# 31415Hacker/RayTracer-public

Measured on AMD Instinct MI355X. Metric: Msamples/sec @1920x1080 Stanford-Dragon-class, 4 spp, 8 bounces, higher is better.
Workload: dtype f32; 1 GPU; C2: dragon-class procedural closed mesh (871414 tris, seed 20260109; dragon.glb absent), native LBVH2->BVH4, 1920x1080, 4 spp, 8 bounces, camera (0,0,2.5) identity quat FOV 70, a new frame index (sample set) every step; triangles=871414, bvh4_nodes=1263056, width=1920, height=1080, spp=4, max_bounces=8, seed=1, frames_per_launch=32

## Files before the change

include/mi355pt.h:

```cpp
#ifndef MI355PT_H
#define MI355PT_H

#include <stdint.h>

#ifdef __cplusplus
extern "C" {
#endif

#if defined(__GNUC__)
#define PT_API __attribute__((visibility("default")))
#else
#define PT_API
#endif

typedef struct PtContext PtContext;

typedef enum PtStatus {
    PT_OK = 0,
    PT_ERR_INVALID_ARG = 1,
    PT_ERR_NO_DEVICE = 2,
    PT_ERR_HIP = 3,
    PT_ERR_NO_SCENE = 4,
    PT_ERR_BAD_BVH = 5,
    PT_ERR_IO = 6,
// ... 183 lines not shown
PT_API int  pt_group_update_triangles(PtGroup* group, const float* tris, uint32_t num_tris);
PT_API int  pt_group_build_bvh(PtGroup* group);
PT_API int  pt_group_build_bvh_accel(PtGroup* group, uint32_t accel);
PT_API int  pt_group_set_bvh2(PtGroup* group, const uint32_t* bvh2, uint64_t words);
PT_API int  pt_group_set_bvh4(PtGroup* group, const uint32_t* bvh4, uint64_t words);
PT_API int  pt_group_set_batch(PtGroup* group, uint32_t frames_per_launch);
PT_API int  pt_group_render(PtGroup* group, const PtRenderParams* params);
PT_API int  pt_group_flush(PtGroup* group);
PT_API int  pt_group_synchronize(PtGroup* group);
PT_API int  pt_group_read_radiance(PtGroup* group, float* dst, uint64_t dst_floats);
PT_API int  pt_group_read_rgba8(PtGroup* group, uint8_t* dst, uint64_t dst_bytes);
PT_API int  pt_group_read_tonemapped(PtGroup* group, int from_rgba8, uint8_t* dst, uint64_t dst_bytes);

PT_API int pt_debug_set_tune(PtContext* ctx, const char* name, uint32_t value);
PT_API int pt_debug_launch_plan(uint32_t num_cus, uint32_t frames, uint32_t tile_count, uint32_t launches_in_flight, uint32_t traced_batches, uint32_t batch_size, uint32_t out[12]);
PT_API int pt_debug_counters(PtContext* ctx, unsigned long long* dst24);
PT_API int pt_debug_wave_times(PtContext* ctx, unsigned long long* dst, uint32_t max_waves, uint32_t* n_waves);
PT_API int pt_debug_traced_tiles(PtContext* ctx, const PtRenderParams* params, uint32_t* bitmask_out, uint32_t words, uint32_t* rect_tiles, uint32_t* traced_tiles);

#ifdef __cplusplus
}
#endif
#endif
```

raytracer-public_amd/__init__.py:

```python
import ctypes as C
import math
import os
import sys

import numpy as np

_HERE = os.path.dirname(os.path.abspath(__file__))
LIB_PATH = os.path.join(_HERE, "libmi355pt.so")

PT_MODE_REFERENCE_PACKET, PT_MODE_REFERENCE, PT_MODE_PATH = 0, 1, 2
PT_FLAG_STATS = 1
PT_FLAG_SIMPLE_KERNEL = 2
PT_FLAG_BRUTE_FORCE = 4
PT_FLAG_COMPACT = 8
SCENE_DRAGON_CLASS, SCENE_SPONZA_CLASS = 0, 1
PT_ACCEL_REFERENCE, PT_ACCEL_AREA_COLLAPSE, PT_ACCEL_PLOC = 0, 1, 2
PT_TRACE_ANY_HIT, PT_TRACE_STATS, PT_TRACE_SIMPLE_KERNEL = 1, 2, 4
PT_CLOSEST_STATS, PT_CLOSEST_SIMPLE_KERNEL, PT_CLOSEST_BRUTE_FORCE = 1, 2, 4
PT_OCCLUSION_STATS, PT_OCCLUSION_SIMPLE_KERNEL = 1, 2
PRIM_NONE = 0xFFFFFFFF


class PtError(RuntimeError):
    def __init__(self, code, message):
# ... 61 lines not shown
    "pt_compute_bvh2_sizing", "pt_compute_bvh4_sizing", "pt_morton_sort", "pt_collapse_lbvh2_to_bvh4",
    "pt_collapse_bvh2_to_bvh4_accel", "pt_build_bvh2_ploc", "pt_bvh2_to_bvh4_wide", "pt_file_write_u32", "pt_file_read_u32", "pt_scene_procedural",
    "pt_set_triangles", "pt_build_bvh", "pt_build_bvh_accel", "pt_build_lbvh2", "pt_read_bvh2", "pt_set_bvh4", "pt_set_bvh2",
    "pt_read_bvh4", "pt_set_spheres", "pt_scene_info", "pt_render", "pt_last_render_ms", "pt_set_batch", "pt_flush", "pt_timing_begin", "pt_timing_collect", "pt_timing_collect_spans", "pt_set_compact_buffer", "pt_set_output_buffer", "pt_get_stats", "pt_read_radiance",
    "pt_read_rgba8", "pt_read_tonemapped", "pt_tile_layout", "pt_tile_ids", "pt_compact_radiance", "pt_deinterleave", "pt_deinterleave_batch", "pt_buffer_busy",
    "pt_accum_info", "pt_read_accum", "pt_set_accum",
    "pt_trace_rays", "pt_trace_rays_host", "pt_camera_rays",
    "pt_closest_points", "pt_closest_points_host", "pt_closest_points_bvh4",
    "pt_occlusion", "pt_occlusion_host", "pt_occlusion_rays", "pt_occlusion_rays_host", "pt_hit_surfels", "pt_hit_surfels_host",
    "pt_update_triangles", "pt_update_triangles_device", "pt_bvh_cost", "pt_refit_bvh4", "pt_refit_bvh2", "pt_bvh4_cost", "pt_group_update_triangles",
    "pt_traced_tile_rect", "pt_packed_layout", "pt_packed_tile_ids", "pt_pack_shares", "pt_unpack_batch",
    "pt_group_create", "pt_group_destroy", "pt_group_last_error", "pt_group_size", "pt_group_context", "pt_group_set_triangles", "pt_group_build_bvh",
    "pt_group_build_bvh_accel",
    "pt_group_set_bvh2", "pt_group_set_bvh4", "pt_group_set_batch", "pt_group_render", "pt_group_flush", "pt_group_synchronize", "pt_group_read_radiance",
    "pt_group_read_rgba8", "pt_group_read_tonemapped",
    "pt_debug_set_tune", "pt_debug_counters", "pt_debug_wave_times", "pt_debug_launch_plan", "pt_debug_traced_tiles",
]


def _load():
    os.environ.setdefault("GPU_MAX_HW_QUEUES", "12")
    if not os.path.exists(LIB_PATH):
        raise ImportError(
            "libmi355pt.so is not built (%s). Run `python -c 'import __graft_entry__ as g; g.build()'` "
            "or `make -C raytracer-public_amd/csrc`. There is no CPU fallback." % LIB_PATH)
    lib = C.CDLL(LIB_PATH)
    lib.pt_last_error.restype = C.c_char_p
    lib.pt_last_error.argtypes = [C.c_void_p]
    lib.pt_version.restype = C.c_char_p
    lib.pt_destroy.restype = None
    lib.pt_destroy.argtypes = [C.c_void_p]
# ... 840 lines not shown
```

raytracer-public_amd/csrc/pt_api.cpp:

```cpp
#include "mi355pt.h"
#include "pt_host.h"
#include "pt_kernels.h"

#include <hip/hip_runtime.h>

#include <algorithm>
#include <cstdio>
#include <cstdlib>
#include <cstring>
#include <string>
#include <vector>

namespace {

thread_local std::string g_global_error;

template <typename T>
struct DevBuf {
    T* ptr = nullptr; size_t cap = 0;
    hipError_t ensure(size_t n) {
        if (n <= cap && ptr) return hipSuccess;
        if (ptr) { (void)hipFree(ptr); ptr = nullptr; cap = 0; }
        if (n == 0) n = 1;
        hipError_t e = hipMalloc((void**)&ptr, n * sizeof(T));
        if (e == hipSuccess) cap = n;
        return e;
    }
    void release() { if (ptr) (void)hipFree(ptr); ptr = nullptr; cap = 0; }
};

}

struct PtTune {
    static constexpr uint32_t kAuto = 0xFFFFFFFFu;
    uint32_t grid_div = kAuto, rows = kAuto, chunk = kAuto, xcd = kAuto, shade = kAuto, fill = kAuto,
             slots = kAuto, cull = kAuto, stats_batch = kAuto, quad = kAuto, fork = kAuto, bounded = kAuto, timeline = kAuto;
    uint32_t* find(const char* name) {
        static const struct { const char* n; uint32_t PtTune::* m; } tab[] = {
            {"GRIDDIV", &PtTune::grid_div}, {"ROWS", &PtTune::rows}, {"CHUNK", &PtTune::chunk}, {"XCD", &PtTune::xcd}, {"SHADE", &PtTune::shade},
            {"FILL", &PtTune::fill}, {"SLOTS", &PtTune::slots}, {"CULL", &PtTune::cull}, {"STATSBATCH", &PtTune::stats_batch}, {"QUAD", &PtTune::quad}, {"FORK", &PtTune::fork}, {"BOUNDED", &PtTune::bounded}, {"TIMELINE", &PtTune::timeline}};
        for (const auto& t : tab) if (std::strcmp(name, t.n) == 0) return &(this->*(t.m));
        return nullptr;
    }
    void from_environment() {
        static const char* names[] = {"GRIDDIV", "ROWS", "CHUNK", "XCD", "SHADE", "FILL", "SLOTS", "CULL", "STATSBATCH", "QUAD", "FORK", "BOUNDED", "TIMELINE"};
        for (const char* n : names) {
            const std::string key = std::string("PT_TUNE_") + n;
            const char* v = std::getenv(key.c_str());
            if (v && *v) *find(n) = uint32_t(std::strtoul(v, nullptr, 10));
        }
    }
    static uint32_t pick(uint32_t knob, uint32_t dflt) { return knob == kAuto ? dflt : knob; }
};

struct PtContext {
    int device = 0;
    PtTune tune;
    hipStream_t own_stream = nullptr;
    hipStream_t stream = nullptr;
    hipEvent_t ev_start = nullptr, ev_stop = nullptr;
// ... 63 lines not shown
    float4* ext_compact = nullptr; uint64_t ext_compact_floats = 0;
    float4* ext_out = nullptr; uint64_t ext_out_floats = 0;
    const float4* last_full = nullptr;
    bool last_stats = false;
    uint64_t stats_culled = 0;
    std::vector<hipEvent_t> ring;
    uint32_t ring_used = 0;
    struct InFlight { const char* lo; const char* hi; uint64_t seq; };
    std::vector<InFlight> inflight;
    uint64_t launch_seq = 0, delivered_seq = 0;
    hipEvent_t misc_fence = nullptr; uint64_t misc_fence_seq = 0;
};

namespace {

int fail(PtContext* ctx, int code, const std::string& msg) {
    if (ctx) ctx->err = msg; else g_global_error = msg;
    return code;
}
int fail_hip(PtContext* ctx, hipError_t e, const char* what) {
    return fail(ctx, PT_ERR_HIP, std::string(what) + ": " + hipGetErrorString(e));
}
#define PT_HIP(ctx, call) do { hipError_t e__ = (call); if (e__ != hipSuccess) return fail_hip((ctx), e__, #call); } while (0)

int bind(PtContext* ctx) {
    if (!ctx) return fail(nullptr, PT_ERR_INVALID_ARG, "null context");
    PT_HIP(ctx, hipSetDevice(ctx->device));
    return PT_OK;
}

// ... 60 lines not shown
    PT_HIP(ctx, hipMalloc((void**)&fresh, tri_bytes + (cap_nodes + 1u) * 64u));
    if (ctx->d_scene.ptr && ctx->scene_tris == num_tris && num_tris)
        PT_HIP(ctx, hipMemcpy(fresh, ctx->d_scene.ptr, uint64_t(num_tris) * 64u, hipMemcpyDeviceToDevice));
    if (ctx->d_scene.ptr) (void)hipFree(ctx->d_scene.ptr);
    PT_HIP(ctx, hipMemset((char*)fresh + uint64_t(num_tris) * 64u, 0, tri_bytes - uint64_t(num_tris) * 64u));
    ctx->d_scene.ptr = fresh; ctx->d_scene.cap = size_t((tri_bytes + (cap_nodes + 1u) * 64u) / 16u);
    ctx->node_off = tri_bytes; ctx->node_cap = cap_nodes; ctx->scene_tris = num_tris;
    return PT_OK;
}

int install_cut(PtContext* ctx) {
    ++ctx->tree_version; ctx->cut_count = 0;
    const uint32_t base16 = uint32_t(ctx->node_off / 16u), root = ctx->wide_meta.root_ref;
    if (root == pt::kInvalid || (root & pt::kLeafFlag) || ctx->num_wide == 0u || root < base16) return PT_OK;
    PT_HIP(ctx, ctx->d_cut.ensure(ptk::kCutMax + 1u));
    if (!ctx->h_word) PT_HIP(ctx, hipHostMalloc((void**)&ctx->h_word, 64, hipHostMallocDefault));
    PT_HIP(ctx, ptk::launch_tile_cut(ctx->wide(), ctx->num_wide, base16, (root - base16) / 4u, ctx->d_cut.ptr, ctx->stream));
    PT_HIP(ctx, hipMemcpyAsync(ctx->h_word, ctx->d_cut.ptr + ptk::kCutMax, 4, hipMemcpyDeviceToHost, ctx->stream));
    PT_HIP(ctx, hipStreamSynchronize(ctx->stream));
    ctx->cut_count = std::min(ctx->h_word[0], ptk::kCutMax);
    return PT_OK;
}

int upload_wide(PtContext* ctx, const uint32_t* bvh4, uint64_t words) {
    pt::WideBvh w; std::string err;
    if (int rc = sync_refit_meta(ctx)) return rc;
    const uint32_t tris_now = ctx->have_tris ? ctx->num_tris : 0u;
    if (!pt::build_wide_bvh(bvh4, words, tris_now, uint32_t(tri_region_bytes(tris_now) / 16u), w, err)) return fail(ctx, PT_ERR_BAD_BVH, err);
    PT_HIP(ctx, ctx->d_bvh4.ensure(words));
    PT_HIP(ctx, hipMemcpyAsync(ctx->d_bvh4.ptr, bvh4, words * 4, hipMemcpyHostToDevice, ctx->stream));
    if (int rc = ensure_scene(ctx, tris_now, w.nodes.size())) return rc;
// ... 50 lines not shown

struct PlanInput {
    uint32_t num_cus;
    uint32_t frames;
    uint32_t tile_count;
    bool     sharded;
    bool     stats;
    uint32_t launches_in_flight;
    uint32_t traced_batches;
    uint32_t batch_size;
};
struct LaunchPlan {
    uint32_t grid;
    uint32_t perm_rows, perm_cols, total_items, chunk_items, xcd_span;
    uint32_t shade_threshold, fill_threshold, quad_live, fork_shadow;
    int      slots, setup_slots;
    const char* error;
};

int slots_for(const PtTune& tune, uint32_t frames, uint32_t tile_count, bool sharded) {
    const uint32_t w8 = frames * 8u / (tile_count ? tile_count : 1u);
    const int n = int(PtTune::pick(tune.slots, w8 >= 256u ? 3u : (w8 >= 64u ? 4u : (w8 >= 16u ? PT_FRAME_SLOTS : (w8 >= 8u ? (sharded ? 4u : 6u) : (sharded ? 8u : PT_FRAME_SLOTS))))));
    return n < 1 ? 1 : (n > PtContext::kMaxSlots ? PtContext::kMaxSlots : n);
}

LaunchPlan plan_launch(const PtTune& tune, const PlanInput& in) {
    LaunchPlan P; std::memset(&P, 0, sizeof(P));
    const uint32_t nf = in.frames, count = in.tile_count ? in.tile_count : 1u;
    const int cus = in.num_cus > 0 ? int(in.num_cus) : 256;
    P.grid = ptk::megakernel_grid(cus);
// ... 6 lines not shown
    const uint32_t work8 = nf * 8u / count;
    P.perm_rows = PtTune::pick(tune.rows, work8 >= 24u ? nf : (work8 >= 8u ? 128u * nf : 64u * nf));
    if (P.perm_rows < 1u) P.perm_rows = 1u;
    if (P.perm_rows > 4096u) P.perm_rows = 4096u;
    P.perm_cols = (in.traced_batches + P.perm_rows - 1u) / P.perm_rows;
    if (uint64_t(P.perm_cols) * P.perm_rows * 64ull > 0xFFFFFFFFull) { P.error = "pt_render: batch too large (more than 2^32 items per launch)"; return P; }
    P.total_items = P.perm_cols * P.perm_rows * 64u;
    P.chunk_items = ((PtTune::pick(tune.chunk, 128u) + 63u) / 64u) * 64u;
    if (P.chunk_items < 64u) P.chunk_items = 64u;
    if (uint64_t(P.total_items) + uint64_t(grid_lanes / 64u + 1u) * P.chunk_items > 0xFFFFFFFFull) {
        P.error = "pt_render: launch too large for the 32-bit work-queue cursor (more than 2^32 - grid * chunk items; lower spp, the resolution or the batch)"; return P;
    }
    {
        const uint32_t per = (P.total_items + 7u) / 8u;
        P.xcd_span = PtTune::pick(tune.xcd, work8 >= 64u ? 1u : 0u) ? ((per + P.chunk_items - 1u) / P.chunk_items) * P.chunk_items : 0u;
    }
    P.shade_threshold = PtTune::pick(tune.shade, PT_SHADE_THRESHOLD); P.fill_threshold = PtTune::pick(tune.fill, PT_FILL_THRESHOLD);
    P.quad_live = std::min(16u, PtTune::pick(tune.quad, PT_QUAD_LIVE));
    P.fork_shadow = PtTune::pick(tune.fork, PT_FORK_SHADOW);
    P.slots = in.stats ? 1 : slots_for(tune, nf, count, in.sharded);
    P.setup_slots = in.stats ? 1 : std::max(P.slots, slots_for(tune, std::max(nf, in.batch_size), count, in.sharded));
    return P;
}

bool launch_rect(const PtContext* ctx, const ptk::FrameParams* frames, uint32_t nf, uint32_t width, uint32_t height, uint32_t num_tris, TileRect& rect) {
    rect = {0, 0, 0, 0};
    if (!(ctx->have_bvh && ctx->wide_meta.root_ref != pt::kInvalid && !ctx->wide_meta.root_degenerate && num_tris != 0u && ctx->tune.cull != 0u)) return false;
    for (uint32_t i = 0; i < nf; ++i) {
        TileRect r;
        if (!root_box_rect(ctx->wide_meta, frames[i], width, height, r)) return false;
// ... 48 lines not shown
        cv.cams = cams; cv.tree_version = ctx->tree_version; cv.width = width; cv.height = height;
        if (!now) return PT_OK;
    }
    if (!cv.computed) {
        if (int rc = sync_refit_meta(ctx)) return rc;
        const uint32_t tiles = ((width + pt::kTile - 1) / pt::kTile) * ((height + pt::kTile - 1) / pt::kTile), words = (tiles + 31u) / 32u;
        if (!ctx->cover_stream) {
            int lo = 0, hi = 0;
            (void)hipDeviceGetStreamPriorityRange(&lo, &hi);
            PT_HIP(ctx, hipStreamCreateWithPriority(&ctx->cover_stream, hipStreamNonBlocking, hi));
        }
        PT_HIP(ctx, ctx->d_cover.ensure(words + 1u));
        if (ctx->h_cover_cap < words + 1u) {
            if (ctx->h_cover) (void)hipHostFree(ctx->h_cover);
            ctx->h_cover = nullptr; ctx->h_cover_cap = 0;
            PT_HIP(ctx, hipHostMalloc((void**)&ctx->h_cover, (size_t(words) + 1u) * sizeof(uint32_t), hipHostMallocDefault));
            ctx->h_cover_cap = words + 1u;
        }
        cv.valid = false;
        PT_HIP(ctx, hipMemsetAsync(ctx->d_cover.ptr, 0, (size_t(words) + 1u) * sizeof(uint32_t), ctx->cover_stream));
        for (size_t first = 0; first < cams.size(); first += ptk::kCoverCams) {
            ptk::CoverCams group; std::memset(&group, 0, sizeof group);
            const uint32_t n = uint32_t(std::min<size_t>(ptk::kCoverCams, cams.size() - first));
            std::memcpy(group.c, cams.data() + first, n * sizeof(ptk::CoverCam));
            PT_HIP(ctx, ptk::launch_tile_cover(ctx->wide(), ctx->d_cut.ptr, ctx->cut_count, group, n, width, height, ctx->d_cover.ptr, words, ctx->cover_stream));
        }
        PT_HIP(ctx, hipMemcpyAsync(ctx->h_cover, ctx->d_cover.ptr, (size_t(words) + 1u) * sizeof(uint32_t), hipMemcpyDeviceToHost, ctx->cover_stream));
        PT_HIP(ctx, hipStreamSynchronize(ctx->cover_stream));
        cv.mask.assign(ctx->h_cover, ctx->h_cover + words);
        cv.usable = ctx->h_cover[words] == 0u;
        cv.id = ++ctx->cover_ids; if (cv.id == 0u) cv.id = ++ctx->cover_ids;
// ... 26 lines not shown
            PT_HIP(ctx, ptk::launch_prime(s.queue.ptr, s.side));
            s.primed_ptr = s.samples.ptr; s.primed_samples = cap_samples;
        }
    }
    return PT_OK;
}

int stage_traced_tiles(PtContext* ctx, PtContext::FrameSlot& sl, const uint32_t key[9], const std::vector<uint32_t>& traced, const uint32_t* cover, uint32_t words) {
    if (sl.cull_valid && std::memcmp(key, sl.cull_key, 9 * sizeof(uint32_t)) == 0) return PT_OK;
    if (!sl.trace_copied) PT_HIP(ctx, hipEventCreateWithFlags(&sl.trace_copied, hipEventDisableTiming));
    else PT_HIP(ctx, hipEventSynchronize(sl.trace_copied));
    const size_t need = traced.size() + words;
    if (sl.h_trace_cap < need) {
        if (sl.h_trace) (void)hipHostFree(sl.h_trace);
        sl.h_trace = nullptr; sl.h_trace_cap = 0;
        PT_HIP(ctx, hipHostMalloc((void**)&sl.h_trace, std::max<size_t>(need, 1024) * sizeof(uint32_t), hipHostMallocDefault));
        sl.h_trace_cap = std::max<size_t>(need, 1024);
    }
    PT_HIP(ctx, sl.trace_slots.ensure(std::max<size_t>(need, 1)));
    if (!traced.empty()) std::memcpy(sl.h_trace, traced.data(), traced.size() * sizeof(uint32_t));
    if (cover) std::memcpy(sl.h_trace + traced.size(), cover, size_t(words) * sizeof(uint32_t));
    else std::memset(sl.h_trace + traced.size(), 0xff, size_t(words) * sizeof(uint32_t));
    sl.cull_valid = false;
    return PT_OK;
}

int flush_pending_stats(PtContext* ctx, bool stats, bool sharded, uint32_t count) {
    if (!ctx->pending) return PT_OK;
    ptk::RenderArgs A = ctx->pendingA;
    const uint32_t nf = ctx->pending;
    ctx->pending = 0;
    const bool ring = ctx->ring_used + 2 <= ctx->ring.size();
    hipEvent_t e0 = ring ? ctx->ring[ctx->ring_used] : ctx->ev_start, e1 = ring ? ctx->ring[ctx->ring_used + 1] : ctx->ev_stop;
    A.num_frames = nf;
    if (uint64_t(A.num_tiles) * A.spp * nf * 64ull > 0xFFFFFFFFull)
        return fail(ctx, PT_ERR_INVALID_ARG, "pt_render: more than 2^32 pixel-samples in one launch (lower spp, the resolution or the batch)");
    A.batches_per_frame = A.num_tiles * A.spp;
    A.num_sample_batches = A.batches_per_frame * nf;
// ... 18 lines not shown
    A.trace_bpf = A.num_trace_tiles * A.spp;
    A.num_batches = A.trace_bpf * nf;
    auto magic = [](uint32_t d) { return d > 1u ? uint32_t(0x100000000ull / d) : 0xFFFFFFFFu; };
    A.trace_bpf_magic = magic(A.trace_bpf ? A.trace_bpf : 1u); A.spp_magic = magic(A.spp); A.tiles_x_magic = magic(A.tiles_x);
    if (A.num_batches == 0u) { A.trace_bpf = 1u; A.trace_bpf_magic = magic(1u); }
    PlanInput in; std::memset(&in, 0, sizeof(in));
    in.num_cus = uint32_t(ctx->num_cus > 0 ? ctx->num_cus : 256); in.frames = nf; in.tile_count = count; in.sharded = sharded; in.stats = stats;
    in.traced_batches = A.num_batches; in.batch_size = ctx->batch_size;
    if (count < 2u && nf == 1u && !stats) {
        for (const auto& o : ctx->slots) if (o.side && o.used && hipEventQuery(o.done) == hipErrorNotReady) ++in.launches_in_flight;
        (void)hipGetLastError();
    }
    const LaunchPlan P = plan_launch(ctx->tune, in);
    if (P.error) return fail(ctx, PT_ERR_INVALID_ARG, P.error);
    A.perm_rows = P.perm_rows; A.perm_rows_magic = magic(P.perm_rows); A.perm_cols = P.perm_cols; A.total_items = P.total_items;
    A.chunk_items = P.chunk_items; A.xcd_span = P.xcd_span;
    A.shade_threshold = P.shade_threshold; A.fill_threshold = P.fill_threshold; A.quad_live = P.quad_live; A.fork_shadow = P.fork_shadow;
    A.rcp_short = (PtTune::pick(ctx->tune.bounded, 1u) != 0u && arith_is_bounded(ctx, ctx->pending_frames, nf)) ? 1u : 0u;

    ctx->num_slots = P.slots;
    if (int rc = prepare_slots(ctx, P, A, nf, stats)) return rc;
    PtContext::FrameSlot& sl = ctx->slots[stats ? 0 : (ctx->next_slot++ % uint32_t(P.slots))];
    A.prime = stats ? 1u : 0u;
    A.samples = sl.samples.ptr; A.queue = sl.queue.ptr; A.spill = sl.spill.ptr; A.raybuf = sl.rays.ptr;
    A.trace_slots = nullptr;
    const uint32_t cull_key[9] = {rect.tx0, rect.ty0, rect.tx1, rect.ty1, A.width, A.height, ctx->pending_rank | (ctx->pending_count << 16), A.num_trace_tiles, cover_id};
    const uint32_t cover_words = (A.tiles_x * ((A.height + pt::kTile - 1) / pt::kTile) + 31u) / 32u;
    if (cull) { if (int rc = stage_traced_tiles(ctx, sl, cull_key, traced, cover, cover_words)) return rc; }
    const bool timeline = !stats && PtTune::pick(ctx->tune.timeline, 0u) != 0u;
    if (stats || timeline) {
        const uint32_t stat_waves = P.grid * ptk::megakernel_block() / 64u;
        PT_HIP(ctx, ctx->d_wave_times.ensure(size_t(stat_waves) * ptk::kWaveTimeWords));
        A.wave_times = ctx->d_wave_times.ptr; ctx->wave_times_n = stat_waves;
    }

    if (!ring) PT_HIP(ctx, hipEventRecord(e0, ctx->stream));
    if (sl.used) PT_HIP(ctx, hipStreamWaitEvent(sl.side, sl.resolved, 0));
    if (cull) {
        if (!sl.cull_valid) {
            PT_HIP(ctx, hipMemcpyAsync(sl.trace_slots.ptr, sl.h_trace, (traced.size() + cover_words) * sizeof(uint32_t), hipMemcpyHostToDevice, sl.side));
            PT_HIP(ctx, hipEventRecord(sl.trace_copied, sl.side));
            std::memcpy(sl.cull_key, cull_key, sizeof cull_key); sl.cull_valid = true; sl.num_trace_tiles = A.num_trace_tiles;
        }
// ... 317 lines not shown
    PT_HIP(ctx, ptk::launch_refit2(ctx->d_tris9.ptr, ctx->num_tris, ctx->d_bvh2.ptr, nn2, ctx->d_refit_parent2.ptr, ctx->d_refit_arrive2.ptr, ctx->stream));
    ctx->bvh2_stale = false; ctx->bvh2_refit_pending = false;
    return PT_OK;
}

int update_triangles(PtContext* ctx, const char* fn, const void* tris, uint32_t num_tris, bool from_device) {
    if (int rc = bind(ctx)) return rc;
    if (!tris) return fail(ctx, PT_ERR_INVALID_ARG, std::string(fn) + ": null triangles");
    if (from_device && (reinterpret_cast<uintptr_t>(tris) & 15u)) return fail(ctx, PT_ERR_INVALID_ARG, std::string(fn) + ": the device array must be 16-byte aligned");
    if (!ctx->have_tris) return fail(ctx, PT_ERR_NO_SCENE, std::string(fn) + ": no triangles uploaded (pt_set_triangles first)");
    if (num_tris != ctx->num_tris) return fail(ctx, PT_ERR_INVALID_ARG, std::string(fn) + ": an update keeps the triangle count (pt_set_triangles changes it)");
    if (int rc = flush_pending(ctx)) return rc;
    if (num_tris == 0u) return PT_OK;
    const bool tree = ctx->have_bvh && ctx->num_nodes4 != 0u;
    if (tree) { if (int rc = ensure_refit_plan(ctx)) return rc; }
    if (!ctx->h_refit) PT_HIP(ctx, hipHostMalloc((void**)&ctx->h_refit, 16, hipHostMallocDefault));
    if (!ctx->ev_refit) PT_HIP(ctx, hipEventCreateWithFlags(&ctx->ev_refit, hipEventDisableTiming));
    PT_HIP(ctx, ctx->d_edge_max.ensure(1));
    PT_HIP(ctx, hipMemsetAsync(ctx->d_edge_max.ptr, 0, sizeof(uint32_t), ctx->stream));
    PT_HIP(ctx, hipMemcpyAsync(ctx->d_tris9.ptr, tris, size_t(num_tris) * 36, from_device ? hipMemcpyDeviceToDevice : hipMemcpyHostToDevice, ctx->stream));
    PT_HIP(ctx, ptk::launch_tri_records(ctx->d_tris9.ptr, num_tris, ctx->trirec(), ctx->d_edge_max.ptr, ctx->stream));
    if (tree) {
        PT_HIP(ctx, ptk::launch_refit4(ctx->d_tris9.ptr, num_tris, ctx->d_bvh4.ptr, ctx->num_nodes4, refit_buffers(ctx), ctx->wide(), ctx->stream));
        PT_HIP(ctx, hipMemcpyAsync(ctx->h_refit, ctx->d_bvh4.ptr + 1, 12, hipMemcpyDeviceToHost, ctx->stream));
        ++ctx->tree_version;
    }
    PT_HIP(ctx, hipMemcpyAsync(ctx->h_refit + 3, ctx->d_edge_max.ptr, 4, hipMemcpyDeviceToHost, ctx->stream));
    PT_HIP(ctx, hipEventRecord(ctx->ev_refit, ctx->stream));
    ctx->meta_pending = true; ctx->meta_has_root = tree;
    if (ctx->have_bvh2) ctx->bvh2_stale = true;
    ctx->accum_count = 0;
// ... 100 lines not shown
    uint32_t nn2 = 0; uint64_t bytes2 = 0;
    pt_compute_bvh2_sizing(n, &nn2, &bytes2);
    PT_HIP(ctx, ctx->d_bvh2.ensure(bytes2 / 4));
    PT_HIP(ctx, ctx->d_morton.ensure(n)); PT_HIP(ctx, ctx->d_triidx.ensure(n));
    PT_HIP(ctx, ctx->d_parent.ensure(nn2)); PT_HIP(ctx, ctx->d_flags.ensure(n > 1 ? n - 1 : 1));
    PT_HIP(ctx, ctx->d_bounds.ensure(6)); PT_HIP(ctx, ctx->d_counters.ensure(ptk::kBuildCounters));
    PT_HIP(ctx, ctx->d_code_tmp.ensure(n)); PT_HIP(ctx, ctx->d_index_tmp.ensure(n));
    PT_HIP(ctx, ctx->d_node2.ensure(nn2)); PT_HIP(ctx, ctx->d_child_pos.ensure(nn2)); PT_HIP(ctx, ctx->d_subtree.ensure(nn2));
    PT_HIP(ctx, ctx->d_ids.ensure(nn2)); PT_HIP(ctx, ctx->d_bnd.ensure(size_t(nn2) * 3));
    size_t temp_bytes = ptk::build_temp_bytes(n);
    if (accel == PT_ACCEL_PLOC) {
        temp_bytes = std::max(temp_bytes, ptk::ploc_temp_bytes(n));
        PT_HIP(ctx, ctx->d_ploc.ensure(ptk::ploc_words(n)));
    }
    PT_HIP(ctx, ctx->d_build_temp.ensure(temp_bytes));
    if (!ctx->h_word) PT_HIP(ctx, hipHostMalloc((void**)&ctx->h_word, 64, hipHostMallocDefault));
    PT_HIP(ctx, ctx->d_bvh4.ensure(1 + size_t(nn2) * 8));
    ptk::BuildBuffers B;
    B.bounds = ctx->d_bounds.ptr; B.counters = ctx->d_counters.ptr; B.code_tmp = ctx->d_code_tmp.ptr; B.index_tmp = ctx->d_index_tmp.ptr;
    B.morton = ctx->d_morton.ptr; B.tri_index = ctx->d_triidx.ptr; B.temp = ctx->d_build_temp.ptr; B.temp_bytes = temp_bytes;
    B.node2 = ctx->d_node2.ptr; B.child_pos = ctx->d_child_pos.ptr; B.subtree = ctx->d_subtree.ptr; B.ids = ctx->d_ids.ptr; B.bnd = ctx->d_bnd.ptr;
    B.host_word = ctx->h_word;
    ctx->have_bvh = false; ctx->have_bvh2 = false;
    ctx->refit_ready = false; ctx->refit2_ready = false; ctx->bvh2_stale = false;
    PT_HIP(ctx, hipMemcpyAsync(ctx->d_bvh2.ptr, &nn2, 4, hipMemcpyHostToDevice, ctx->stream));
    PT_HIP(ctx, ptk::launch_morton_sort(B, ctx->d_tris9.ptr, n, ctx->stream));
    if (accel == PT_ACCEL_PLOC) {
        uint32_t iterations = 0;
        hipError_t e = ptk::build_ploc_on_device(B, ctx->d_ploc.ptr, ctx->d_tris9.ptr, n, ctx->d_bvh2.ptr, ctx->d_parent.ptr, ctx->d_flags.ptr, &iterations, ctx->stream);
        if (e == hipErrorInvalidValue) return fail(ctx, PT_ERR_BAD_BVH, "pt_build_bvh_accel: a PLOC iteration merged no pair");
        PT_HIP(ctx, e);
// ... 572 lines not shown
}

int pt_debug_launch_plan(uint32_t num_cus, uint32_t frames, uint32_t tile_count, uint32_t launches_in_flight, uint32_t traced_batches, uint32_t batch_size, uint32_t out[12]) {
    if (!out || frames == 0u) return fail(nullptr, PT_ERR_INVALID_ARG, "pt_debug_launch_plan: bad arguments");
    PlanInput in; std::memset(&in, 0, sizeof(in));
    in.num_cus = num_cus; in.frames = frames; in.tile_count = tile_count ? tile_count : 1u; in.sharded = in.tile_count > 1u; in.stats = false;
    in.launches_in_flight = launches_in_flight; in.traced_batches = traced_batches; in.batch_size = batch_size ? batch_size : 1u;
    const LaunchPlan P = plan_launch(PtTune(), in);
    if (P.error) return fail(nullptr, PT_ERR_INVALID_ARG, P.error);
    const uint32_t v[12] = {P.grid, P.perm_rows, P.perm_cols, P.total_items, P.chunk_items, P.xcd_span, P.shade_threshold, P.fill_threshold, P.quad_live, P.fork_shadow,
                            uint32_t(P.slots), uint32_t(P.setup_slots)};
    std::memcpy(out, v, sizeof v);
    return PT_OK;
}

int pt_debug_counters(PtContext* ctx, unsigned long long* dst24) {
    if (int rc = bind(ctx)) return rc;
    PT_HIP(ctx, hipMemcpy(dst24, ctx->d_stats.ptr, 24 * sizeof(unsigned long long), hipMemcpyDeviceToHost));
    return PT_OK;
}

int pt_debug_wave_times(PtContext* ctx, unsigned long long* dst, uint32_t max_waves, uint32_t* n_waves) {
    if (int rc = bind(ctx)) return rc;
    const uint32_t n = ctx->wave_times_n < max_waves ? ctx->wave_times_n : max_waves;
    if (n) PT_HIP(ctx, hipMemcpy(dst, ctx->d_wave_times.ptr, size_t(n) * ptk::kWaveTimeWords * 8u, hipMemcpyDeviceToHost));
    if (n_waves) *n_waves = n;
    return PT_OK;
}

int pt_debug_traced_tiles(PtContext* ctx, const PtRenderParams* p, uint32_t* bitmask_out, uint32_t words, uint32_t* rect_tiles, uint32_t* traced_tiles_out) {
// ... 305 lines not shown
```

raytracer-public_amd/csrc/pt_kernels.h:

```cpp
#pragma once
#include <hip/hip_runtime.h>
#include <stdint.h>

#define PT_KMODE_PACKET    0
#define PT_KMODE_REFERENCE 1
#define PT_KMODE_PATH      2

#ifndef PT_SHORT_STACK
#define PT_SHORT_STACK 12
#endif
#ifndef PT_MEGA_WAVES_PER_SIMD
#define PT_MEGA_WAVES_PER_SIMD 6
#endif
#ifndef PT_FRAME_SLOTS
#define PT_FRAME_SLOTS 3
#endif
#ifndef PT_MEGA_BLOCK
#define PT_MEGA_BLOCK 64
#endif
#ifndef PT_SHADE_THRESHOLD
#define PT_SHADE_THRESHOLD 16
#endif
#ifndef PT_QUAD
#define PT_QUAD 1
// ... 21 lines not shown
#endif
#ifndef PT_PQ_WAVES_PER_SIMD
#define PT_PQ_WAVES_PER_SIMD 6
#endif
#ifndef PT_PQ_FILL
#define PT_PQ_FILL 8
#endif
#ifndef PT_OC_SHORT_STACK
#define PT_OC_SHORT_STACK 12
#endif
#ifndef PT_OC_WAVES_PER_SIMD
#define PT_OC_WAVES_PER_SIMD 6
#endif
#ifndef PT_OC_FILL
#define PT_OC_FILL 8
#endif
#ifndef PT_FILL_THRESHOLD
#define PT_FILL_THRESHOLD 4
#endif

namespace ptk {

constexpr int kStackMax = 64;
constexpr uint32_t kWaveTimeWords = 24;
#define PT_MAX_BATCH 256
struct FrameParams {
    float cam[3]; float focal;
    float quat[4];
    float aspect; uint32_t frame; uint32_t seed;
    uint32_t accum_mode;
};
constexpr int kFrameChunk = 32;
struct FrameChunk { FrameParams f[kFrameChunk]; float4* o[kFrameChunk]; };

struct RenderArgs {
    const uint4*  nodes;
    const float4* tris;
    const uint4*  scene;
    uint32_t      node_off;
    uint32_t      rcp_short;
    uint32_t      tri_gate;
    const uint32_t* bvh4_ref;
    const float*    tris9;
    float4*   out;
    float4*   accum;
    uint32_t* tri_ids;
// ... 8 lines not shown
    uint32_t frame;
    uint32_t root_ref; uint32_t root_box[3]; uint32_t root_degenerate;
    uint32_t spp, max_bounces, seed, accumulate, compact;
    float4*   samples;
    uint32_t* queue;
    uint2*    spill;
    uint4*    raybuf;
    unsigned long long* wave_times;
    const uint32_t* trace_slots; uint32_t num_trace_tiles;
    uint32_t  trace_rect[4];
    uint32_t  trace_bpf, trace_bpf_magic;
    uint32_t  spp_magic, tiles_x_magic;
    uint32_t  num_sample_batches;
    uint32_t  total_items, chunk_items;
    uint32_t  xcd_span;
    uint32_t  num_batches, perm_cols;
    uint32_t  perm_rows, perm_rows_magic;
    uint32_t  shade_threshold, fill_threshold;
    uint32_t  fork_shadow;
    uint32_t  quad_live;
    const FrameParams* frames; float4* const* outs;
    uint32_t  num_frames, batches_per_frame;
    uint32_t  prime;
    uint32_t  ref_mode;
};

hipError_t launch_render(const RenderArgs& args, int kmode, bool stats, hipStream_t stream);
hipError_t launch_trace(const RenderArgs& args, bool stats, uint32_t grid_blocks, hipStream_t stream, hipEvent_t k0, hipEvent_t k1);
hipError_t launch_prime(uint32_t* queue, hipStream_t stream);
hipError_t launch_frame_params(const FrameParams* frames, float4* const* outs, uint32_t n, FrameParams* d_frames, float4** d_outs, hipStream_t stream);
// ... 69 lines not shown
```

raytracer-public_amd/csrc/pt_megakernel.hip:

```cpp
#include <hip/hip_runtime.h>
#include <stdint.h>

#include "pt_kernels.h"
#include "pt_device.h"

namespace ptk {

#ifndef PT_TAIL_PRIORITY
#define PT_TAIL_PRIORITY 3
#endif
#define PT_TAIL_PRIO do { if (PT_TAIL_PRIORITY) __builtin_amdgcn_s_setprio(PT_TAIL_PRIORITY); } while (0)
constexpr int kShort = PT_SHORT_STACK;
constexpr uint32_t kPhaseIdle = 0, kPhaseTrav = 1, kPhaseDone = 2, kPhaseWait = 3;
struct Lane {
    F3 o, d, inv;
    RaySel sel;
    float best_t; uint32_t best_tri;
    uint32_t cur; int sp;
    F3 T, rad;
    F3 d_next, contrib;
    uint32_t key, item;
    uint32_t bounce;
};

// ... 93 lines not shown
        if (scene_is_empty()) return false;
        if (STATS && count_lane()) { c_nodes += 1; if (c_maxstack < 1u) c_maxstack = 1u; }
        if (A.root_degenerate != 0u) return false;
        Ray r; r.o = S.o; r.d = S.d; r.inv = S.inv;
        float troot;
        if (!slab(r, A.root_box[0], A.root_box[1], A.root_box[2], kInfT, troot)) return false;
        if (STATS && count_lane()) ++c_enter;
        S.cur = A.root_ref;
        S.sel = ray_selectors(S.inv);
        return true;
    };

    uint4* const rb = A.raybuf + ((size_t)blockIdx.x * (PT_MEGA_BLOCK / 64) + wave) * (64 * 3);
    uint32_t rb_next = 0, rb_count = 0;
    auto source_dry = [&]() __attribute__((always_inline)) -> bool { return queue_empty && rb_next == rb_count; };
    auto claim_chunk = [&]() __attribute__((always_inline)) {
        if (A.xcd_span != 0u) {
            for (;;) {
                const uint32_t qi = (xcc + xcd_hop) & 7u;
                const uint32_t q_begin = qi * A.xcd_span;
                const uint32_t q_end = min(q_begin + A.xcd_span, total_items);
                uint32_t start = 0;
                if (lane == 0) start = atomicAdd(A.queue + 8 + qi, chunk_items);
                start = __builtin_amdgcn_readfirstlane(start);
                if (q_begin < q_end && start < q_end - q_begin) { chunk_next = q_begin + start; chunk_end = min(chunk_next + chunk_items, q_end); break; }
                if (++xcd_hop == 8u) { queue_empty = true; PT_TAIL_PRIO; if (TIMELINE) tl_event(1, 6, 8, 15); break; }
            }
        } else {
            uint32_t start = 0;
            if (lane == 0) start = atomicAdd(A.queue, chunk_items);
            start = __builtin_amdgcn_readfirstlane(start);
            if (start >= total_items) { queue_empty = true; PT_TAIL_PRIO; if (TIMELINE) tl_event(1, 6, 8, 15); }
            else { chunk_next = start; chunk_end = min(start + chunk_items, total_items); }
        }
    };
    auto shade_due = [&](unsigned long long m_live) __attribute__((always_inline)) -> uint32_t {
        if (!source_dry()) return A.shade_threshold;
        const uint32_t q = (uint32_t)__popcll(m_live) >> 2;
        return q < 1u ? 1u : (q < A.shade_threshold ? q : A.shade_threshold);
    };
    bool want_reseat = false;
    auto reseat = [&]() __attribute__((always_inline)) {
        const unsigned long long m_live = __ballot(phase != kPhaseIdle);
        const uint32_t n_live = (uint32_t)__popcll(m_live);
        uint32_t srcl = lane;
        {
            unsigned long long m = m_live; uint32_t r = 0u;
            while (m != 0ull) {
// ... 206 lines not shown
```

raytracer-public_amd/csrc/pt_megakernel_loop.inc:

```
    constexpr bool quad = PT_LOOP_QUAD != 0;
    uint32_t ref_mode = A.ref_mode;
    asm volatile("" : "+s"(ref_mode));
    for (;;) {
        {
            const unsigned long long m_done = __ballot(phase == kPhaseDone);
            const unsigned long long m_trav = __ballot(phase == kPhaseTrav);
            if (m_done != 0ull && ((uint32_t)__popcll(m_done) >= shade_due(m_trav | m_done) || m_trav == 0ull)) {
                if (TIMELINE) ++n_shade;
                if (STATS) cy_mark = __builtin_amdgcn_s_memtime();
                if (ref_mode) {
                    if (phase == kPhaseDone) {
                        const F3 col = base * (0.15f + wmax(dot3(tri_normal_ref(A, S.best_tri), L), 0.0f));
                        A.samples[S.item] = make_float4(col.x, col.y, col.z, 1.0f);
                        phase = kPhaseIdle;
                    }
                } else {
                const bool fork_on = PT_LOOP_FORK;
                bool want_fork = false;
                if (fork_on) {
                    const int ca = (int)((S.bounce >> kChildShift) << 2);
                    const uint32_t c_phase = (uint32_t)__builtin_amdgcn_ds_bpermute(ca, (int)phase), c_tri = (uint32_t)__builtin_amdgcn_ds_bpermute(ca, (int)S.best_tri);
                    if (STATS) {
                        const uint32_t c_bounce = (uint32_t)__builtin_amdgcn_ds_bpermute(ca, (int)S.bounce);
                        if ((S.bounce & kPendBit) && (c_phase == kPhaseIdle || (c_bounce & kForkedBit) == 0u)) atomicOr(&A.stats[7], 1ull << 63);
// ... 107 lines not shown
            const uint32_t n_live = (uint32_t)__popcll(__ballot(phase != kPhaseIdle));
            if (__builtin_expect(n_live != 0u && n_live <= A.quad_live, 0)) { want_reseat = true; break; }
        }
        {
            const unsigned long long m_idle = __ballot(phase == kPhaseIdle);
            const unsigned long long m_trav = __ballot(phase == kPhaseTrav);
            if ((quad || PT_LOOP_STAGE == 0) && m_idle != 0ull && !source_dry() && ((uint32_t)__popcll(m_idle) >= A.fill_threshold || m_trav == 0ull)) {
                const uint32_t want = (uint32_t)__popcll(m_idle) >> (quad ? 2 : 0);
                const uint32_t rank = lanes_below(m_idle) >> (quad ? 2 : 0);
                if (TIMELINE) ++n_fill;
                if (STATS) cy_mark = __builtin_amdgcn_s_memtime();
                {
                    while (rb_next == rb_count && !queue_empty) {
                        if (chunk_next == chunk_end) claim_chunk();
                        if (queue_empty) break;
                        const uint32_t first = chunk_next; chunk_next += 64u;
                        const ItemInfo it = decode_item(A, first + lane);
                        bool enters = false; Ray r; uint32_t key = 0u;
                        r.o = r.d = r.inv = f3(0.0f, 0.0f, 0.0f);
                        if (it.valid) {
                            float bgp = 0.0f + 1.0f * kBgPrimary;
                            asm volatile("" : "+v"(bgp));
                            A.samples[it.sample_index] = make_float4(bgp, bgp, bgp, 1.0f);
                            const FrameParams fp = frames[it.fid];
                            if (ref_mode) r = primary_ray_fp<BOUNDED>(A, fp, (float)it.px + 0.5f, (float)it.py + 0.5f);
                            else {
                                key = sample_key(fp.seed, it.py * A.width + it.px, fp.frame * A.spp + it.s);
                                r = primary_ray_fp<BOUNDED>(A, fp, (float)it.px + rnd(key, 0, 0), (float)it.py + rnd(key, 0, 1));
                            }
                            if (STATS) { ++c_closest; ++c_samples; }
                            if (!scene_is_empty()) {
                                if (STATS) { c_nodes += 1; if (c_maxstack < 1u) c_maxstack = 1u; }
                                float troot;
                                if (A.root_degenerate == 0u) enters = slab(r, A.root_box[0], A.root_box[1], A.root_box[2], kInfT, troot);
                            }
// ... 257 lines not shown
```

Baseline: 12860 Msamples/s.

## Add tapered work-queue chunk sizes and pre-stage cull tables for idle slots

```diff
diff --git a/include/mi355pt.h b/include/mi355pt.h
--- a/include/mi355pt.h
+++ b/include/mi355pt.h
@@ -221,6 +221,9 @@
 
 PT_API int pt_debug_set_tune(PtContext* ctx, const char* name, uint32_t value);
 PT_API int pt_debug_launch_plan(uint32_t num_cus, uint32_t frames, uint32_t tile_count, uint32_t launches_in_flight, uint32_t traced_batches, uint32_t batch_size, uint32_t out[12]);
+PT_API int pt_debug_queue_plan(uint32_t num_cus, uint32_t frames, uint32_t tile_count, uint32_t launches_in_flight, uint32_t traced_batches, uint32_t batch_size, uint32_t taper,
+                               uint32_t plan[16], uint32_t* chunks, uint64_t max_chunks, uint64_t* n_chunks);
+PT_API int pt_debug_alloc_count(uint64_t* count);
 PT_API int pt_debug_counters(PtContext* ctx, unsigned long long* dst24);
 PT_API int pt_debug_wave_times(PtContext* ctx, unsigned long long* dst, uint32_t max_waves, uint32_t* n_waves);
 PT_API int pt_debug_traced_tiles(PtContext* ctx, const PtRenderParams* params, uint32_t* bitmask_out, uint32_t words, uint32_t* rect_tiles, uint32_t* traced_tiles);
diff --git a/raytracer-public_amd/__init__.py b/raytracer-public_amd/__init__.py
--- a/raytracer-public_amd/__init__.py
+++ b/raytracer-public_amd/__init__.py
@@ -99,7 +99,7 @@
     "pt_group_build_bvh_accel",
     "pt_group_set_bvh2", "pt_group_set_bvh4", "pt_group_set_batch", "pt_group_render", "pt_group_flush", "pt_group_synchronize", "pt_group_read_radiance",
     "pt_group_read_rgba8", "pt_group_read_tonemapped",
-    "pt_debug_set_tune", "pt_debug_counters", "pt_debug_wave_times", "pt_debug_launch_plan", "pt_debug_traced_tiles",
+    "pt_debug_set_tune", "pt_debug_counters", "pt_debug_wave_times", "pt_debug_launch_plan", "pt_debug_traced_tiles", "pt_debug_queue_plan", "pt_debug_alloc_count",
 ]
 
 
diff --git a/raytracer-public_amd/csrc/pt_api.cpp b/raytracer-public_amd/csrc/pt_api.cpp
--- a/raytracer-public_amd/csrc/pt_api.cpp
+++ b/raytracer-public_amd/csrc/pt_api.cpp
@@ -5,6 +5,7 @@
 #include <hip/hip_runtime.h>
 
 #include <algorithm>
+#include <atomic>
 #include <cstdio>
 #include <cstdlib>
 #include <cstring>
@@ -14,6 +15,7 @@
 namespace {
 
 thread_local std::string g_global_error;
+std::atomic<uint64_t> g_alloc_count{0};
 
 template <typename T>
 struct DevBuf {
@@ -23,6 +25,7 @@
         if (ptr) { (void)hipFree(ptr); ptr = nullptr; cap = 0; }
         if (n == 0) n = 1;
         hipError_t e = hipMalloc((void**)&ptr, n * sizeof(T));
+        ++g_alloc_count;
         if (e == hipSuccess) cap = n;
         return e;
     }
@@ -34,16 +37,16 @@
 struct PtTune {
     static constexpr uint32_t kAuto = 0xFFFFFFFFu;
     uint32_t grid_div = kAuto, rows = kAuto, chunk = kAuto, xcd = kAuto, shade = kAuto, fill = kAuto,
-             slots = kAuto, cull = kAuto, stats_batch = kAuto, quad = kAuto, fork = kAuto, bounded = kAuto, timeline = kAuto;
+             slots = kAuto, cull = kAuto, stats_batch = kAuto, quad = kAuto, fork = kAuto, bounded = kAuto, timeline = kAuto, taper = kAuto;
     uint32_t* find(const char* name) {
         static const struct { const char* n; uint32_t PtTune::* m; } tab[] = {
             {"GRIDDIV", &PtTune::grid_div}, {"ROWS", &PtTune::rows}, {"CHUNK", &PtTune::chunk}, {"XCD", &PtTune::xcd}, {"SHADE", &PtTune::shade},
-            {"FILL", &PtTune::fill}, {"SLOTS", &PtTune::slots}, {"CULL", &PtTune::cull}, {"STATSBATCH", &PtTune::stats_batch}, {"QUAD", &PtTune::quad}, {"FORK", &PtTune::fork}, {"BOUNDED", &PtTune::bounded}, {"TIMELINE", &PtTune::timeline}};
+            {"FILL", &PtTune::fill}, {"SLOTS", &PtTune::slots}, {"CULL", &PtTune::cull}, {"STATSBATCH", &PtTune::stats_batch}, {"QUAD", &PtTune::quad}, {"FORK", &PtTune::fork}, {"BOUNDED", &PtTune::bounded}, {"TIMELINE", &PtTune::timeline}, {"TAPER", &PtTune::taper}};
         for (const auto& t : tab) if (std::strcmp(name, t.n) == 0) return &(this->*(t.m));
         return nullptr;
     }
     void from_environment() {
-        static const char* names[] = {"GRIDDIV", "ROWS", "CHUNK", "XCD", "SHADE", "FILL", "SLOTS", "CULL", "STATSBATCH", "QUAD", "FORK", "BOUNDED", "TIMELINE"};
+        static const char* names[] = {"GRIDDIV", "ROWS", "CHUNK", "XCD", "SHADE", "FILL", "SLOTS", "CULL", "STATSBATCH", "QUAD", "FORK", "BOUNDED", "TIMELINE", "TAPER"};
         for (const char* n : names) {
             const std::string key = std::string("PT_TUNE_") + n;
             const char* v = std::getenv(key.c_str());
@@ -137,6 +140,8 @@
 
 namespace {
 
+hipError_t pinned_alloc(void** p, size_t bytes) { ++g_alloc_count; return hipHostMalloc(p, bytes, hipHostMallocDefault); }
+
 int fail(PtContext* ctx, int code, const std::string& msg) {
     if (ctx) ctx->err = msg; else g_global_error = msg;
     return code;
@@ -227,7 +232,7 @@
     const uint32_t base16 = uint32_t(ctx->node_off / 16u), root = ctx->wide_meta.root_ref;
     if (root == pt::kInvalid || (root & pt::kLeafFlag) || ctx->num_wide == 0u || root < base16) return PT_OK;
     PT_HIP(ctx, ctx->d_cut.ensure(ptk::kCutMax + 1u));
-    if (!ctx->h_word) PT_HIP(ctx, hipHostMalloc((void**)&ctx->h_word, 64, hipHostMallocDefault));
+    if (!ctx->h_word) PT_HIP(ctx, pinned_alloc((void**)&ctx->h_word, 64));
     PT_HIP(ctx, ptk::launch_tile_cut(ctx->wide(), ctx->num_wide, base16, (root - base16) / 4u, ctx->d_cut.ptr, ctx->stream));
     PT_HIP(ctx, hipMemcpyAsync(ctx->h_word, ctx->d_cut.ptr + ptk::kCutMax, 4, hipMemcpyDeviceToHost, ctx->stream));
     PT_HIP(ctx, hipStreamSynchronize(ctx->stream));
@@ -308,6 +313,8 @@
     uint32_t grid;
     uint32_t perm_rows, perm_cols, total_items, chunk_items, xcd_span;
     uint32_t shade_threshold, fill_threshold, quad_live, fork_shadow;
+    uint32_t taper_floor, taper_waves;
+    ptk::ClaimZones claim;
     int      slots, setup_slots;
     const char* error;
 };
@@ -344,6 +351,13 @@
     {
         const uint32_t per = (P.total_items + 7u) / 8u;
         P.xcd_span = PtTune::pick(tune.xcd, work8 >= 64u ? 1u : 0u) ? ((per + P.chunk_items - 1u) / P.chunk_items) * P.chunk_items : 0u;
+    }
+    {
+        const uint32_t waves = grid_lanes / 64u;
+        const uint32_t floor = PtTune::pick(tune.taper, PT_TAPER_FLOOR);
+        P.taper_floor = floor == 0u || floor >= 128u || P.chunk_items != 128u ? 0u : (floor <= 16u && P.xcd_span != 0u ? 16u : (floor <= 32u ? 32u : 64u));
+        P.taper_waves = P.xcd_span ? std::max(1u, waves / 8u) : std::max(1u, waves);
+        P.claim = ptk::claim_zones(P.xcd_span ? P.xcd_span : P.total_items, P.taper_waves, P.chunk_items, P.taper_floor);
     }
     P.shade_threshold = PtTune::pick(tune.shade, PT_SHADE_THRESHOLD); P.fill_threshold = PtTune::pick(tune.fill, PT_FILL_THRESHOLD);
     P.quad_live = std::min(16u, PtTune::pick(tune.quad, PT_QUAD_LIVE));
@@ -422,7 +436,7 @@
         if (ctx->h_cover_cap < words + 1u) {
             if (ctx->h_cover) (void)hipHostFree(ctx->h_cover);
             ctx->h_cover = nullptr; ctx->h_cover_cap = 0;
-            PT_HIP(ctx, hipHostMalloc((void**)&ctx->h_cover, (size_t(words) + 1u) * sizeof(uint32_t), hipHostMallocDefault));
+            PT_HIP(ctx, pinned_alloc((void**)&ctx->h_cover, (size_t(words) + 1u) * sizeof(uint32_t)));
             ctx->h_cover_cap = words + 1u;
         }
         cv.valid = false;
@@ -479,7 +493,7 @@
     if (sl.h_trace_cap < need) {
         if (sl.h_trace) (void)hipHostFree(sl.h_trace);
         sl.h_trace = nullptr; sl.h_trace_cap = 0;
-        PT_HIP(ctx, hipHostMalloc((void**)&sl.h_trace, std::max<size_t>(need, 1024) * sizeof(uint32_t), hipHostMallocDefault));
+        PT_HIP(ctx, pinned_alloc((void**)&sl.h_trace, std::max<size_t>(need, 1024) * sizeof(uint32_t)));
         sl.h_trace_cap = std::max<size_t>(need, 1024);
     }
     PT_HIP(ctx, sl.trace_slots.ensure(std::max<size_t>(need, 1)));
@@ -487,6 +501,20 @@
     if (cover) std::memcpy(sl.h_trace + traced.size(), cover, size_t(words) * sizeof(uint32_t));
     else std::memset(sl.h_trace + traced.size(), 0xff, size_t(words) * sizeof(uint32_t));
     sl.cull_valid = false;
+    return PT_OK;
+}
+
+int stage_fresh_slots(PtContext* ctx, const LaunchPlan& P, const PtContext::FrameSlot* current, const uint32_t key[9], const std::vector<uint32_t>& traced,
+                      const uint32_t* cover, uint32_t words, uint32_t num_trace_tiles) {
+    for (int si = 0; si < P.setup_slots; ++si) {
+        PtContext::FrameSlot& s = ctx->slots[si];
+        if (&s == current || s.used || !s.side) continue;
+        if (s.cull_valid && std::memcmp(key, s.cull_key, 9 * sizeof(uint32_t)) == 0) continue;
+        if (int rc = stage_traced_tiles(ctx, s, key, traced, cover, words)) return rc;
+        PT_HIP(ctx, hipMemcpyAsync(s.trace_slots.ptr, s.h_trace, (traced.size() + words) * sizeof(uint32_t), hipMemcpyHostToDevice, s.side));
+        PT_HIP(ctx, hipEventRecord(s.trace_copied, s.side));
+        std::memcpy(s.cull_key, key, 9 * sizeof(uint32_t)); s.cull_valid = true; s.num_trace_tiles = num_trace_tiles;
+    }
     return PT_OK;
 }
 
@@ -535,7 +563,7 @@
     const LaunchPlan P = plan_launch(ctx->tune, in);
     if (P.error) return fail(ctx, PT_ERR_INVALID_ARG, P.error);
     A.perm_rows = P.perm_rows; A.perm_rows_magic = magic(P.perm_rows); A.perm_cols = P.perm_cols; A.total_items = P.total_items;
-    A.chunk_items = P.chunk_items; A.xcd_span = P.xcd_span;
+    A.chunk_items = P.chunk_items; A.xcd_span = P.xcd_span; A.claim = P.claim;
     A.shade_threshold = P.shade_threshold; A.fill_threshold = P.fill_threshold; A.quad_live = P.quad_live; A.fork_shadow = P.fork_shadow;
     A.rcp_short = (PtTune::pick(ctx->tune.bounded, 1u) != 0u && arith_is_bounded(ctx, ctx->pending_frames, nf)) ? 1u : 0u;
 
@@ -548,6 +576,7 @@
     const uint32_t cull_key[9] = {rect.tx0, rect.ty0, rect.tx1, rect.ty1, A.width, A.height, ctx->pending_rank | (ctx->pending_count << 16), A.num_trace_tiles, cover_id};
     const uint32_t cover_words = (A.tiles_x * ((A.height + pt::kTile - 1) / pt::kTile) + 31u) / 32u;
     if (cull) { if (int rc = stage_traced_tiles(ctx, sl, cull_key, traced, cover, cover_words)) return rc; }
+    if (cull && !stats) { if (int rc = stage_fresh_slots(ctx, P, &sl, cull_key, traced, cover, cover_words, A.num_trace_tiles)) return rc; }
     const bool timeline = !stats && PtTune::pick(ctx->tune.timeline, 0u) != 0u;
     if (stats || timeline) {
         const uint32_t stat_waves = P.grid * ptk::megakernel_block() / 64u;
@@ -895,7 +924,7 @@
     if (num_tris == 0u) return PT_OK;
     const bool tree = ctx->have_bvh && ctx->num_nodes4 != 0u;
     if (tree) { if (int rc = ensure_refit_plan(ctx)) return rc; }
-    if (!ctx->h_refit) PT_HIP(ctx, hipHostMalloc((void**)&ctx->h_refit, 16, hipHostMallocDefault));
+    if (!ctx->h_refit) PT_HIP(ctx, pinned_alloc((void**)&ctx->h_refit, 16));
     if (!ctx->ev_refit) PT_HIP(ctx, hipEventCreateWithFlags(&ctx->ev_refit, hipEventDisableTiming));
     PT_HIP(ctx, ctx->d_edge_max.ensure(1));
     PT_HIP(ctx, hipMemsetAsync(ctx->d_edge_max.ptr, 0, sizeof(uint32_t), ctx->stream));
@@ -1026,7 +1055,7 @@
         PT_HIP(ctx, ctx->d_ploc.ensure(ptk::ploc_words(n)));
     }
     PT_HIP(ctx, ctx->d_build_temp.ensure(temp_bytes));
-    if (!ctx->h_word) PT_HIP(ctx, hipHostMalloc((void**)&ctx->h_word, 64, hipHostMallocDefault));
+    if (!ctx->h_word) PT_HIP(ctx, pinned_alloc((void**)&ctx->h_word, 64));
     PT_HIP(ctx, ctx->d_bvh4.ensure(1 + size_t(nn2) * 8));
     ptk::BuildBuffers B;
     B.bounds = ctx->d_bounds.ptr; B.counters = ctx->d_counters.ptr; B.code_tmp = ctx->d_code_tmp.ptr; B.index_tmp = ctx->d_index_tmp.ptr;
@@ -1629,6 +1658,44 @@
     return PT_OK;
 }
 
+int pt_debug_queue_plan(uint32_t num_cus, uint32_t frames, uint32_t tile_count, uint32_t launches_in_flight, uint32_t traced_batches, uint32_t batch_size, uint32_t taper,
+                        uint32_t plan[16], uint32_t* chunks, uint64_t max_chunks, uint64_t* n_chunks) {
+    if (!plan || frames == 0u) return fail(nullptr, PT_ERR_INVALID_ARG, "pt_debug_queue_plan: bad arguments");
+    PlanInput in; std::memset(&in, 0, sizeof(in));
+    in.num_cus = num_cus; in.frames = frames; in.tile_count = tile_count ? tile_count : 1u; in.sharded = in.tile_count > 1u; in.stats = false;
+    in.launches_in_flight = launches_in_flight; in.traced_batches = traced_batches; in.batch_size = batch_size ? batch_size : 1u;
+    PtTune tune; tune.taper = taper;
+    const LaunchPlan P = plan_launch(tune, in);
+    if (P.error) return fail(nullptr, PT_ERR_INVALID_ARG, P.error);
+    const uint32_t ranges = P.xcd_span ? 8u : 1u;
+    const uint32_t v[16] = {P.total_items, P.chunk_items, P.xcd_span, ranges, P.taper_waves, P.taper_floor, P.claim.c1, P.claim.c2, P.claim.c3, P.claim.b1, P.claim.b2, P.claim.b3,
+                            P.grid * ptk::megakernel_block() / 64u, 0u, 0u, 0u};
+    std::memcpy(plan, v, sizeof v);
+    uint64_t n = 0;
+    for (uint32_t qi = 0; qi < ranges; ++qi) {
+        const uint64_t q_begin = P.xcd_span ? uint64_t(qi) * P.xcd_span : 0u;
+        const uint64_t q_end = P.xcd_span ? std::min<uint64_t>(q_begin + P.xcd_span, P.total_items) : P.total_items;
+        if (q_begin >= q_end) continue;
+        for (uint32_t c = 0;; ++c) {
+            uint32_t first, size;
+            ptk::claim_chunk_at(P.claim, P.chunk_items, c, first, size);
+            if (first >= q_end - q_begin) break;
+            if (chunks && n < max_chunks) {
+                chunks[3 * n] = qi; chunks[3 * n + 1] = uint32_t(q_begin) + first; chunks[3 * n + 2] = uint32_t(std::min<uint64_t>(q_begin + first + size, q_end));
+            }
+            ++n;
+        }
+    }
+    if (n_chunks) *n_chunks = n;
+    return PT_OK;
+}
+
+int pt_debug_alloc_count(uint64_t* count) {
+    if (!count) return fail(nullptr, PT_ERR_INVALID_ARG, "pt_debug_alloc_count: null output");
+    *count = g_alloc_count.load();
+    return PT_OK;
+}
+
 int pt_debug_counters(PtContext* ctx, unsigned long long* dst24) {
     if (int rc = bind(ctx)) return rc;
     PT_HIP(ctx, hipMemcpy(dst24, ctx->d_stats.ptr, 24 * sizeof(unsigned long long), hipMemcpyDeviceToHost));
diff --git a/raytracer-public_amd/csrc/pt_kernels.h b/raytracer-public_amd/csrc/pt_kernels.h
--- a/raytracer-public_amd/csrc/pt_kernels.h
+++ b/raytracer-public_amd/csrc/pt_kernels.h
@@ -59,6 +59,9 @@
 #endif
 #ifndef PT_OC_FILL
 #define PT_OC_FILL 8
+#endif
+#ifndef PT_TAPER_FLOOR
+#define PT_TAPER_FLOOR 0
 #endif
 #ifndef PT_FILL_THRESHOLD
 #define PT_FILL_THRESHOLD 4
@@ -75,6 +78,25 @@
     float aspect; uint32_t frame; uint32_t seed;
     uint32_t accum_mode;
 };
+struct ClaimZones { uint32_t c1, c2, c3, b1, b2, b3; };
+__host__ __device__ inline void claim_chunk_at(const ClaimZones& z, uint32_t chunk_items, uint32_t c, uint32_t& first, uint32_t& size) {
+    if (c < z.c1) { first = c * chunk_items; size = chunk_items; }
+    else if (c < z.c2) { first = z.b1 + ((c - z.c1) << 6); size = 64u; }
+    else if (c < z.c3) { first = z.b2 + ((c - z.c2) << 5); size = 32u; }
+    else { first = z.b3 + ((c - z.c3) << 4); size = 16u; }
+}
+inline ClaimZones claim_zones(uint32_t len, uint32_t waves, uint32_t chunk_items, uint32_t floor) {
+    ClaimZones z = {0xFFFFFFFFu, 0xFFFFFFFFu, 0xFFFFFFFFu, 0u, 0u, 0u};
+    if (floor == 0u || floor > 64u || chunk_items != 128u) return z;
+    if (waves < 1u) waves = 1u;
+    auto from = [&](uint32_t s) { const uint64_t tail = 2ull * s * waves; return tail >= len ? 0u : uint32_t((len - tail) & ~127ull); };
+    z.b1 = from(64u); z.b2 = from(32u); z.b3 = from(16u);
+    z.c1 = z.b1 / 128u;
+    if (floor <= 32u) z.c2 = z.c1 + (z.b2 - z.b1) / 64u;
+    if (floor <= 16u) z.c3 = z.c2 + (z.b3 - z.b2) / 32u;
+    return z;
+}
+
 constexpr int kFrameChunk = 32;
 struct FrameChunk { FrameParams f[kFrameChunk]; float4* o[kFrameChunk]; };
 
@@ -113,6 +135,7 @@
     uint32_t  num_sample_batches;
     uint32_t  total_items, chunk_items;
     uint32_t  xcd_span;
+    ClaimZones claim;
     uint32_t  num_batches, perm_cols;
     uint32_t  perm_rows, perm_rows_magic;
     uint32_t  shade_threshold, fill_threshold;
diff --git a/raytracer-public_amd/csrc/pt_megakernel.hip b/raytracer-public_amd/csrc/pt_megakernel.hip
--- a/raytracer-public_amd/csrc/pt_megakernel.hip
+++ b/raytracer-public_amd/csrc/pt_megakernel.hip
@@ -1,5 +1,6 @@
 #include <hip/hip_runtime.h>
 #include <stdint.h>
+#include <stddef.h>
 
 #include "pt_kernels.h"
 #include "pt_device.h"
@@ -131,24 +132,34 @@
     uint4* const rb = A.raybuf + ((size_t)blockIdx.x * (PT_MEGA_BLOCK / 64) + wave) * (64 * 3);
     uint32_t rb_next = 0, rb_count = 0;
     auto source_dry = [&]() __attribute__((always_inline)) -> bool { return queue_empty && rb_next == rb_count; };
+    auto claim_at = [&](uint32_t c, uint32_t& start, uint32_t& size) __attribute__((always_inline)) {
+        typedef const __attribute__((address_space(4))) char* KernArg;
+        KernArg ka = (KernArg)__builtin_amdgcn_kernarg_segment_ptr();
+        asm volatile("" : "+s"(ka));
+        const __attribute__((address_space(4))) uint32_t* zw = (const __attribute__((address_space(4))) uint32_t*)(ka + offsetof(RenderArgs, claim));
+        const ClaimZones z = {zw[0], zw[1], zw[2], zw[3], zw[4], zw[5]};
+        claim_chunk_at(z, chunk_items, c, start, size);
+    };
     auto claim_chunk = [&]() __attribute__((always_inline)) {
         if (A.xcd_span != 0u) {
             for (;;) {
                 const uint32_t qi = (xcc + xcd_hop) & 7u;
                 const uint32_t q_begin = qi * A.xcd_span;
                 const uint32_t q_end = min(q_begin + A.xcd_span, total_items);
-                uint32_t start = 0;
-                if (lane == 0) start = atomicAdd(A.queue + 8 + qi, chunk_items);
-                start = __builtin_amdgcn_readfirstlane(start);
-                if (q_begin < q_end && start < q_end - q_begin) { chunk_next = q_begin + start; chunk_end = min(chunk_next + chunk_items, q_end); break; }
+                uint32_t c = 0, start, size;
+                if (lane == 0) c = atomicAdd(A.queue + 8 + qi, 1u);
+                c = __builtin_amdgcn_readfirstlane(c);
+                claim_at(c, start, size);
+                if (q_begin < q_end && start < q_end - q_begin) { chunk_next = q_begin + start; chunk_end = min(chunk_next + size, q_end); break; }
                 if (++xcd_hop == 8u) { queue_empty = true; PT_TAIL_PRIO; if (TIMELINE) tl_event(1, 6, 8, 15); break; }
             }
         } else {
-            uint32_t start = 0;
-            if (lane == 0) start = atomicAdd(A.queue, chunk_items);
-            start = __builtin_amdgcn_readfirstlane(start);
+            uint32_t c = 0, start, size;
+            if (lane == 0) c = atomicAdd(A.queue, 1u);
+            c = __builtin_amdgcn_readfirstlane(c);
+            claim_at(c, start, size);
             if (start >= total_items) { queue_empty = true; PT_TAIL_PRIO; if (TIMELINE) tl_event(1, 6, 8, 15); }
-            else { chunk_next = start; chunk_end = min(start + chunk_items, total_items); }
+            else { chunk_next = start; chunk_end = min(start + size, total_items); }
         }
     };
     auto shade_due = [&](unsigned long long m_live) __attribute__((always_inline)) -> uint32_t {
diff --git a/raytracer-public_amd/csrc/pt_megakernel_loop.inc b/raytracer-public_amd/csrc/pt_megakernel_loop.inc
--- a/raytracer-public_amd/csrc/pt_megakernel_loop.inc
+++ b/raytracer-public_amd/csrc/pt_megakernel_loop.inc
@@ -145,11 +145,11 @@
                     while (rb_next == rb_count && !queue_empty) {
                         if (chunk_next == chunk_end) claim_chunk();
                         if (queue_empty) break;
-                        const uint32_t first = chunk_next; chunk_next += 64u;
+                        const uint32_t first = chunk_next; chunk_next = min(chunk_next + 64u, chunk_end);
                         const ItemInfo it = decode_item(A, first + lane);
                         bool enters = false; Ray r; uint32_t key = 0u;
                         r.o = r.d = r.inv = f3(0.0f, 0.0f, 0.0f);
-                        if (it.valid) {
+                        if (it.valid & (first + lane < chunk_end)) {
                             float bgp = 0.0f + 1.0f * kBgPrimary;
                             asm volatile("" : "+v"(bgp));
                             A.samples[it.sample_index] = make_float4(bgp, bgp, bgp, 1.0f);
```

After: 12840 Msamples/s. About the same (-0.2%).
